# SketchyScene/SketchySceneColorization

Hardware: AMD Instinct MI355X
Metric: train images/sec (192x192, gen+disc fwd+bwd) (higher is better)
Workload: dtype fp32 (bf16x6 split on the bf16 MFMA, fp32 accumulate; filter gradients and few-channel layers on the exact-fp32 MFMA); 1 GPU; Foreground_Instance_Colorization Pix2Pix GAN train step (D-step + G-step, TF-Adam), 192x192, batch 32 per GPU; global_batch=32, parallelism=dp1, ranks_observed_by_allreduce=1, launcher=in-process, block_type=Pix2Pix, launch=hipGraph replay

## Files before the change

### sketchyscenecolorization_amd/csrc/igemm_bf16.hip

```cpp
#include <hip/hip_runtime.h>
#include <stdint.h>
#include <stdio.h>
#include <stdlib.h>
#include "sketchycolor_hip.h"
#include "igemm_util.h"
#include "igemm_epilogue.h"
#include "host_util.h"

#define BK 32
#ifndef SSC_BF_DIAG_BUILD
#define SSC_BF_DIAG_BUILD 0
#endif
typedef short bf16x8 __attribute__((ext_vector_type(8)));
typedef __bf16 bf16x2_t __attribute__((ext_vector_type(2)));
typedef unsigned u32x2_t __attribute__((ext_vector_type(2)));

__device__ unsigned g_sk_cfg_bf[4] = {2000000000u, 0u, 0u, 0u};

int ssc_sk_configure_bf(const unsigned* cfg4) {
    return (int)hipMemcpyToSymbol(HIP_SYMBOL(g_sk_cfg_bf), cfg4, 4 * sizeof(unsigned), 0, hipMemcpyHostToDevice);
}

template <int N>
__device__ __forceinline__ void glds16_run(const char* sbase, const unsigned* voff, unsigned lds_addr) {
    unsigned keep;
    if (N == 1) {
        asm volatile("s_mov_b32 %0, m0\n\ts_mov_b32 m0, %3\n\ts_nop 0\n\tglobal_load_lds_dwordx4 %1, %2\n\ts_mov_b32 m0, %0"
                     : "=&s"(keep) : "v"(voff[0]), "s"(sbase), "s"(lds_addr) : "memory");
    } else if (N == 2) {
        asm volatile("s_mov_b32 %0, m0\n\ts_mov_b32 m0, %4\n\ts_nop 0\n\tglobal_load_lds_dwordx4 %1, %3\n\t"
                     "s_add_u32 m0, m0, 0x400\n\ts_nop 0\n\tglobal_load_lds_dwordx4 %2, %3\n\ts_mov_b32 m0, %0"
                     : "=&s"(keep) : "v"(voff[0]), "v"(voff[1]), "s"(sbase), "s"(lds_addr) : "memory", "scc");
    } else {
        static_assert(N >= 1 && N <= 3, "1..3 instructions per run");
        asm volatile("s_mov_b32 %0, m0\n\ts_mov_b32 m0, %5\n\ts_nop 0\n\tglobal_load_lds_dwordx4 %1, %4\n\t"
                     "s_add_u32 m0, m0, 0x400\n\ts_nop 0\n\tglobal_load_lds_dwordx4 %2, %4\n\t"
                     "s_add_u32 m0, m0, 0x400\n\ts_nop 0\n\tglobal_load_lds_dwordx4 %3, %4\n\ts_mov_b32 m0, %0"
                     : "=&s"(keep) : "v"(voff[0]), "v"(voff[1]), "v"(voff[2]), "s"(sbase), "s"(lds_addr) : "memory", "scc");
    }
}

__device__ __forceinline__ unsigned cvt_pk_bf16(float a, float b) {
    const f32x2_t v = {a, b};
    return __builtin_bit_cast(unsigned, __builtin_convertvector(v, bf16x2_t));
}
__device__ __forceinline__ void split3_pair(float x0, float x1, unsigned& h, unsigned& m, unsigned& l) {
    if (SSC_BF_DIAG_BUILD & 16) { h = m = l = __float_as_uint(x0) ^ __float_as_uint(x1); return; }
    h = cvt_pk_bf16(x0, x1);
    const float r0 = x0 - __uint_as_float(h << 16), r1 = x1 - __uint_as_float(h & 0xffff0000u);
    m = cvt_pk_bf16(r0, r1);
    const float s0 = r0 - __uint_as_float(m << 16), s1 = r1 - __uint_as_float(m & 0xffff0000u);
    l = cvt_pk_bf16(s0, s1);
}

struct SplitGeom { int K, N, KC, NBP; };
static inline SplitGeom split_geom(int c0, int c1, int orient) {
    SplitGeom g;
    g.K = orient ? c1 : c0;
    g.N = orient ? c0 : c1;
    g.KC = 2 * ((g.K + 31) / 32);
    g.NBP = (g.N + 31) / 32 + 3;
    return g;
}

static int64_t ssc_filter_split_bytes(int taps, int c0, int c1, int orient) {
    const SplitGeom g = split_geom(c0, c1, orient);
    return (int64_t)taps * g.KC * 3 * g.NBP * 1024;
}

__device__ __forceinline__ unsigned rne_bf16_bits(float x) {
    const unsigned u = __float_as_uint(x);
    return (u + 0x7fffu + ((u >> 16) & 1u)) & 0xffff0000u;
}

__device__ __forceinline__ void filter_split_body(const ssc_split_job& jb, long lt) {
    const int K = jb.orient ? jb.c1 : jb.c0, N = jb.orient ? jb.c0 : jb.c1;
    const int KC = 2 * ((K + 31) / 32), NBP = (N + 31) / 32 + 3;
    const long nfrag = (long)jb.taps * KC * NBP;
    if (lt >= nfrag * 64) return;
    const int lane = (int)(lt & 63);
    const long f = lt >> 6;
    const int nb = (int)(f % NBP);
    const long r = f / NBP;
    const int kc = (int)(r % KC), tap = (int)(r / KC);
    const int n = nb * 32 + (lane & 31), k0 = kc * 16 + (lane >> 5) * 8;
    unsigned hb[8], mb[8], lb[8];
#pragma unroll
    for (int e = 0; e < 8; ++e) {
        const int k = k0 + e;
        float x = 0.f;
        if (k < K && n < N)
            x = jb.orient ? jb.w[((long)tap * jb.c0 + n) * jb.c1 + k] : jb.w[((long)tap * jb.c0 + k) * jb.c1 + n];
        const unsigned h = rne_bf16_bits(x);
        const float r1 = x - __uint_as_float(h);
        const unsigned m = rne_bf16_bits(r1);
        const float r2 = r1 - __uint_as_float(m);
        hb[e] = h; mb[e] = m; lb[e] = rne_bf16_bits(r2);
    }
    uint4 vh, vm, vl;
    vh.x = (hb[0] >> 16) | hb[1]; vh.y = (hb[2] >> 16) | hb[3]; vh.z = (hb[4] >> 16) | hb[5]; vh.w = (hb[6] >> 16) | hb[7];
    vm.x = (mb[0] >> 16) | mb[1]; vm.y = (mb[2] >> 16) | mb[3]; vm.z = (mb[4] >> 16) | mb[5]; vm.w = (mb[6] >> 16) | mb[7];
    vl.x = (lb[0] >> 16) | lb[1]; vl.y = (lb[2] >> 16) | lb[3]; vl.z = (lb[4] >> 16) | lb[5]; vl.w = (lb[6] >> 16) | lb[7];
    char* base = reinterpret_cast<char*>(jb.dst) + ((((long)tap * KC + kc) * 3) * NBP + nb) * 1024 + lane * 16;
    *reinterpret_cast<uint4*>(base) = vh;
    *reinterpret_cast<uint4*>(base + (long)NBP * 1024) = vm;
    *reinterpret_cast<uint4*>(base + (long)2 * NBP * 1024) = vl;
}

__global__ __launch_bounds__(256) void filter_split_kernel(const ssc_split_job* __restrict__ jobs, int njobs) {
    const long t = (long)blockIdx.x * 256 + threadIdx.x;
    const long tb = (long)blockIdx.x * 256;
    int lo = 0, hi = njobs - 1;
    while (lo < hi) {
        const int mid = (lo + hi + 1) >> 1;
        if (jobs[mid].first_thread <= tb) lo = mid;
        else hi = mid - 1;
    }
    const ssc_split_job jb = jobs[lo];
    filter_split_body(jb, t - jb.first_thread);
}
__global__ __launch_bounds__(256) void filter_split_one_kernel(const ssc_split_job jb) {
    filter_split_body(jb, (long)blockIdx.x * 256 + threadIdx.x);
}

static int64_t ssc_filter_split_threads(int taps, int c0, int c1, int orient) {
    const SplitGeom g = split_geom(c0, c1, orient);
    return (((int64_t)taps * g.KC * g.NBP * 64 + 255) / 256) * 256;
}

extern "C" int ssc_filter_split_geom(int taps, int c0, int c1, int orient, int* kc, int* nbp, int64_t* bytes, int64_t* threads) {
    if (taps <= 0 || c0 <= 0 || c1 <= 0) return -1;
    const SplitGeom g = split_geom(c0, c1, orient);
    if (kc) *kc = g.KC;
    if (nbp) *nbp = g.NBP;
    if (bytes) *bytes = ssc_filter_split_bytes(taps, c0, c1, orient);
    if (threads) *threads = ssc_filter_split_threads(taps, c0, c1, orient);
    return 0;
}

extern "C" int ssc_filter_split_batch(const ssc_split_job* jobs_dev, int njobs, int64_t total_threads, void* stream) {
    if (njobs <= 0 || total_threads <= 0) return 0;
    if (total_threads / 256 > 0x7fffffffL) return -1;
    hipLaunchKernelGGL(filter_split_kernel, dim3((unsigned)(total_threads / 256)), dim3(256), 0, (hipStream_t)stream, jobs_dev, njobs);
    return (int)hipGetLastError();
}

#define BF_A_RS 208
#define BF_WAIT_ALL() do { asm volatile("s_waitcnt vmcnt(0)" ::: "memory"); __builtin_amdgcn_s_waitcnt(0x0070); } while (0)
template <int BM, int BN, bool SS = false> struct BfLds {
    static constexpr int A_BYTES = BM * BF_A_RS;
    static constexpr int B_BYTES = 6 * (BN / 32) * 1024;
    static constexpr int EPI_BYTES = (BM * (BN + 4) + 2 * 256 * 4) * 4;
    static constexpr int ONE = A_BYTES + B_BYTES;
    static constexpr int OPER_BYTES = SS ? (ONE > EPI_BYTES ? ONE : EPI_BYTES) : 2 * ONE;
    static constexpr int TOTAL = OPER_BYTES + BM * 8;
};

struct BfTabs { const float* a0; const float* b0; const float* a1; const float* b1; };
template <int WM, int WN, int SM, int SN, bool PLAIN, bool ONE, bool KM = false, bool SS = false>
__global__ __launch_bounds__(256) void conv_bf_kernel(const ssc_conv_desc d, const Magics mg, float* __restrict__ slab_base,
                                                       long slab_stride, int splitk, int ts_full, int ts_s,
                                                       unsigned* __restrict__ flags, const BfTabs tab, const int korder) {
    constexpr int BM = WM * SM * 32;
    constexpr int BN = WN * SN * 32;
    constexpr int NBT = BN / 32;
    constexpr int A_BYTES = BfLds<BM, BN, SS>::A_BYTES, B_BYTES = BfLds<BM, BN, SS>::B_BYTES;
    constexpr int LDS_FLOATS = BfLds<BM, BN, SS>::OPER_BYTES / 4;
    constexpr int B_BASE = (SS ? 1 : 2) * A_BYTES;
    constexpr int A_ROWS = BM / 32;
    constexpr int B_IPW = 6 * NBT / 4;
    static_assert(WM * WN == 4 && (6 * NBT) % 4 == 0, "4 waves share the fragments of a K-tile evenly");

    extern __shared__ __attribute__((aligned(16))) float smem[];
    char* const sm_b = reinterpret_cast<char*>(smem);
    long* rowpix = reinterpret_cast<long*>(smem + LDS_FLOATS);

    const int tid = threadIdx.x;
    const int lane = tid & 63;
    const int wave = tid >> 6;
    const int wm = wave / WN, wn = wave % WN;
    const int l31 = lane & 31, lhi = lane >> 5;

    const float* const xs0 = d.x.s0;
    const float* const xs1 = d.x.s1;
    const int xC0 = d.x.C0, xC1 = d.x.C1, xH = d.x.H, xW = d.x.W;
    const int TWv = d.TW, kstep = d.kstep, KWv = d.KW;
    const float slope0 = act_slope(d.x.act), slope1 = act_slope(d.x.act1 >= 0 ? d.x.act1 : d.x.act);

    static_assert(!KM || ONE, "partial chunks: one source only");
    const int nch0 = KM ? (xC0 + BK - 1) / BK : xC0 / BK, nch1 = xC1 / BK;
    const int tpt = nch0 + nch1;
    const long M = (long)d.NB * d.PH * d.PW;
    const int PHW = d.PH * d.PW;
    int phase, ks, sk, n0, slot = 0;
    long m0;
    float* part = nullptr;
    if (ts_s > 0) {
        const int bid = blockIdx.x;
        int tile;
        if (bid < ts_full) {
            tile = bid; ks = 0; sk = 1;
        } else {
            const int r = bid - ts_full;
            const int q = r / (ts_s & 0xffff);
            tile = ts_full + q; ks = r - q * (ts_s & 0xffff); sk = ts_s & 0xffff;
            part = slab_base + (long)r * (BM * BN);
            slot = r;
        }
        const int mt = (int)((M + BM - 1) / BM), nt = (d.Nstore + BN - 1) / BN;
        if (ts_s & 0x10000) {
            if (bid < ts_full) tile = (bid & 7) * (ts_full >> 3) + (bid >> 3);
            const int r2 = tile / nt;
            n0 = (tile - r2 * nt) * BN;
            if (ts_s & 0x20000) {
                phase = r2 & 3;
                m0 = (long)(r2 >> 2) * BM;
            } else {
                phase = r2 / mt;
                m0 = (long)(r2 - phase * mt) * BM;
            }
            ts_s &= 0xffff;
            sk = bid < ts_full ? 1 : ts_s;
        } else {
            const int rest = tile / mt;
            m0 = (long)(tile - rest * mt) * BM;
            phase = rest / nt;
            n0 = (rest - phase * nt) * BN;
        }
    } else {
        phase = blockIdx.z / splitk;
        ks = blockIdx.z % splitk;
// ... 288 lines not shown
                        if (SSC_BF_DIAG_BUILD & 64) { asm volatile("" : "=v"(av[kc][i][p])); continue; }
                        av[kc][i][p] = *reinterpret_cast<const bf16x8*>(Ab + i * 32 * BF_A_RS + p * 64 + kc * 32);
                    }
            };
            auto fetch_b = [&](int kc) {
#pragma unroll
                for (int j = 0; j < SN; ++j)
#pragma unroll
                    for (int p = 0; p < 3; ++p) {
                        if (SSC_BF_DIAG_BUILD & 64) { asm volatile("" : "=v"(bv[kc][j][p])); continue; }
                        bv[kc][j][p] = *reinterpret_cast<const bf16x8*>(Bb + ((kc * 3 + p) * NBT + j) * 1024);
                    }
            };
            auto group = [&](int kc, int t) {
                if (SSC_BF_DIAG_BUILD & 1) return;
                constexpr int pa[6] = {2, 0, 1, 1, 0, 0}, pb[6] = {0, 2, 1, 0, 1, 0};
#pragma unroll
                for (int i = 0; i < SM; ++i)
#pragma unroll
                    for (int j = 0; j < SN; ++j) {
                        if (t == 5)
                            acc[i][j] = __builtin_amdgcn_mfma_f32_32x32x16_bf16(av[kc][i][0], bv[kc][j][0], acc[i][j], 0, 0, 0);
                        else
                            accc[i][j] = __builtin_amdgcn_mfma_f32_32x32x16_bf16(av[kc][i][pa[t]], bv[kc][j][pb[t]], accc[i][j], 0, 0, 0);
                    }
            };
#define BF_SB __builtin_amdgcn_sched_barrier(0)
            fetch_a(0);
            fetch_b(0);
            if (SS) {
                fetch_a(1);
                fetch_b(1);
                asm volatile("s_waitcnt lgkmcnt(0)" ::: "memory");
                __builtin_amdgcn_s_barrier();
            }
            BF_SB;
            float z0, w0, z1, w1;
            unsigned ha, ma, la, hb, mb, lb;
            group(0, 0); dma_b(td, nxt, 0); BF_SB;
            group(0, 1); if (RUN1 > 0) dma_b(td, nxt, 1); BF_SB;
            if (kt + 2 <= last) kt_advance(tl);
            group(0, 2); issue_loads(tl, SB); BF_SB;
            group(0, 3); if (!SS) fetch_a(1); BF_SB;
            group(0, 4); if (!SS) fetch_b(1); BF_SB;
            if (A_ROWS == 2) {
                group(0, 5); BF_STAGE_A(SA, 0, z0, w0, ha, ma, la); BF_SB;
                group(1, 0); BF_STAGE_B(nxt, 0, z0, w0, ha, ma, la); BF_SB;
                group(1, 1); BF_STAGE_A(SA, 1, z1, w1, hb, mb, lb); BF_SB;
                group(1, 2); BF_STAGE_B(nxt, 1, z1, w1, hb, mb, lb); BF_SB;
                group(1, 3); BF_SB;
                group(1, 4); BF_SB;
                group(1, 5); BF_SB;
            } else {
                group(0, 5); BF_STAGE_A(SA, 0, z0, w0, ha, ma, la); BF_SB;
                group(1, 0); BF_STAGE_B(nxt, 0, z0, w0, ha, ma, la); BF_STAGE_A(SA, 1, z1, w1, hb, mb, lb); BF_SB;
                group(1, 1); BF_STAGE_B(nxt, 1, z1, w1, hb, mb, lb); BF_STAGE_A(SA, 2, z0, w0, ha, ma, la); BF_SB;
                group(1, 2); BF_STAGE_B(nxt, 2, z0, w0, ha, ma, la); BF_STAGE_A(SA, 3, z1, w1, hb, mb, lb); BF_SB;
                group(1, 3); BF_STAGE_B(nxt, 3, z1, w1, hb, mb, lb); BF_SB;
                group(1, 4); BF_SB;
                group(1, 5); BF_SB;
            }
#undef BF_SB
            BF_WAIT_ALL();
            td = tl;
            __builtin_amdgcn_s_barrier();
        };
        for (int kt = kt_begin; kt < kt_end; kt += 2) {
            kstep(S0, S1, 0, kt);
            if (kt + 1 < kt_end) kstep(S1, S0, 1, kt + 1);
        }
    }

#pragma unroll
    for (int i = 0; i < SM; ++i)
#pragma unroll
        for (int j = 0; j < SN; ++j)
#pragma unroll
            for (int r = 0; r < 16; ++r) acc[i][j][r] += accc[i][j][r];
    ut_epilogue<BM, BN, WM, WN, SM, SN, LDS_FLOATS>(acc, d, smem, rowpix, part, ks, sk, slot, flags, ts_s, splitk, slab_base,
                                                   slab_stride, m0, n0, phase, M, g_sk_cfg_bf);
}

#define BFH_A_RS 112
template <int BM, int BN> struct BfhLds {
    static constexpr int A_BYTES = BM * BFH_A_RS;
    static constexpr int B_BYTES = 3 * (BN / 32) * 1024;
    static constexpr int OPER_BYTES = 2 * (A_BYTES + B_BYTES);
    static constexpr int EPI_BYTES = (BM * (BN + 4) + 2 * 256 * 4) * 4;
    static constexpr int LDS_BYTES = OPER_BYTES > EPI_BYTES ? OPER_BYTES : EPI_BYTES;
    static constexpr int TOTAL = LDS_BYTES + BM * 8;
};

template <int WM, int WN, bool PLAIN, bool ONE, bool KM = false>
__global__ __launch_bounds__(256, 2) void conv_bfh_kernel(const ssc_conv_desc d, const Magics mg, float* __restrict__ slab_base,
                                                           long slab_stride, int splitk, int ts_full, int ts_s,
                                                           unsigned* __restrict__ flags, const BfTabs tab, const int korder) {
    static_assert(WM * WN == 4, "four waves");
    constexpr int SM = 2, SN = 2, BM = WM * SM * 32, BN = WN * SN * 32, NBT = BN / 32, KS = 16;
    constexpr int A_BYTES = BfhLds<BM, BN>::A_BYTES, B_BYTES = BfhLds<BM, BN>::B_BYTES;
    constexpr int LDS_FLOATS = BfhLds<BM, BN>::LDS_BYTES / 4;
    constexpr int B_BASE = 2 * A_BYTES;
    constexpr int A_ROWS = BM / 64;
    constexpr int B_IPW = 3 * NBT / 4;

    extern __shared__ __attribute__((aligned(16))) float smem[];
    char* const sm_b = reinterpret_cast<char*>(smem);
    long* rowpix = reinterpret_cast<long*>(smem + LDS_FLOATS);

    const int tid = threadIdx.x;
    const int lane = tid & 63;
    const int wave = tid >> 6;
    const int wm = wave / WN, wn = wave % WN;
    const int l31 = lane & 31, lhi = lane >> 5;

    const float* const xs0 = d.x.s0;
    const float* const xs1 = d.x.s1;
    const int xC0 = d.x.C0, xC1 = d.x.C1, xH = d.x.H, xW = d.x.W;
    const int TWv = d.TW, kstep = d.kstep, KWv = d.KW;
    const float slope0 = act_slope(d.x.act), slope1 = act_slope(d.x.act1 >= 0 ? d.x.act1 : d.x.act);

    static_assert(!KM || ONE, "partial chunks: one source only");
    const int nch0 = KM ? (xC0 + KS - 1) / KS : xC0 / KS, nch1 = xC1 / KS;
    const int tpt = nch0 + nch1;
    const long M = (long)d.NB * d.PH * d.PW;
    const int PHW = d.PH * d.PW;
    int phase, ks, sk, n0, slot = 0;
    long m0;
    float* part = nullptr;
    if (ts_s > 0) {
        const int bid = blockIdx.x;
        int tile;
        if (bid < ts_full) {
            tile = bid; ks = 0; sk = 1;
        } else {
            const int r = bid - ts_full;
            const int q = r / (ts_s & 0xffff);
            tile = ts_full + q; ks = r - q * (ts_s & 0xffff); sk = ts_s & 0xffff;
            part = slab_base + (long)r * (BM * BN);
            slot = r;
        }
        const int mt = (int)((M + BM - 1) / BM), nt = (d.Nstore + BN - 1) / BN;
        if (ts_s & 0x10000) {
            if (bid < ts_full) tile = (bid & 7) * (ts_full >> 3) + (bid >> 3);
            const int r2 = tile / nt;
            n0 = (tile - r2 * nt) * BN;
            if (ts_s & 0x20000) {
                phase = r2 & 3;
                m0 = (long)(r2 >> 2) * BM;
            } else {
                phase = r2 / mt;
                m0 = (long)(r2 - phase * mt) * BM;
            }
            ts_s &= 0xffff;
            sk = bid < ts_full ? 1 : ts_s;
        } else {
            const int rest = tile / mt;
            m0 = (long)(tile - rest * mt) * BM;
            phase = rest / nt;
            n0 = (rest - phase * nt) * BN;
        }
    } else {
        phase = blockIdx.z / splitk;
        ks = blockIdx.z % splitk;
        sk = splitk;
        m0 = (long)blockIdx.x * BM;
        n0 = blockIdx.y * BN;
    }
    const FwdPhase ph = fwd_phase(d, phase);

    const int a_col4 = tid & 3;
    const int aq = tid >> 2;
    const int arow = (aq & ~7) | ((aq & 3) << 1) | ((aq >> 2) & 1);
    const bool a_lastv = !KM || (nch0 - 1) * KS + a_col4 * 4 < xC0;
    uint4 a_lastm = make_uint4(~0u, ~0u, ~0u, ~0u);
    if (KM) {
        const int c_ = (nch0 - 1) * KS + a_col4 * 4;
        a_lastm = make_uint4(c_ < d.k_real ? ~0u : 0u, c_ + 1 < d.k_real ? ~0u : 0u, c_ + 2 < d.k_real ? ~0u : 0u,
                             c_ + 3 < d.k_real ? ~0u : 0u);
    }
    int a_iyb[A_ROWS], a_ixb[A_ROWS], a_off0[A_ROWS], a_off1[A_ROWS];
    bool a_mv[A_ROWS];
#pragma unroll
    for (int i = 0; i < A_ROWS; ++i) {
        const int row = arow + 64 * i;
        const long m = m0 + row;
        a_mv[i] = m < M;
// ... 76 lines not shown
            if (korder == 1) {
                t.ty = sidx / TWv;
                t.tx = sidx - t.ty * TWv;
            } else {
                const int hw = TWv >> 1, pc = ntaps >> 2;
                const int cls = sidx / pc, j = sidx - cls * pc;
                const int jy = j / hw, jx = j - jy * hw;
                t.ty = 2 * jy + (cls >> 1);
                t.tx = 2 * jx + (cls & 1);
            }
            kt_place(t);
            return t;
        }
        const int tap = div32(kt, mg.mC, mg.oneC);
        t.chunk = kt - tap * tpt;
        t.ty = div32(tap, mg.mTW, mg.oneTW);
        t.tx = tap - t.ty * TWv;
        kt_place(t);
        return t;
    };
    const long W0 = (long)(ph.ky0 * KWv + ph.kx0) * KC * KB;
    const long SX2 = 2 * SX, DY2 = 2 * SY - (long)TWv * SX;
    auto kt_advance = [&](KTile& t) {
        if (korder == 1) {
            t.tx += 1;
            t.tapidx += 1;
            t.tappix += 1;
            t.woff += SX;
            if (t.tx == TWv) {
                t.tx = 0;
                t.ty += 1;
                t.tappix += xW - TWv;
                t.woff += DY;
                if (t.ty == THv) {
                    t.ty = 0;
                    t.chunk += 1;
                    t.tapidx = 0;
                    t.tappix = 0;
                    t.woff = W0 + (long)t.chunk * KB;
                }
            }
            return;
        }
        if (korder == 2) {
            t.tx += 2;
            t.tapidx += 2;
            t.tappix += 2;
            t.woff += SX2;
            if (t.tx >= TWv) {
                t.tx -= TWv;
                t.ty += 2;
                t.tapidx += TWv;
                t.tappix += 2 * xW - TWv;
                t.woff += DY2;
                if (t.ty >= THv) {
                    t.ty &= 1;
                    if (t.tx == 0) t.tx = 1;
                    else {
                        t.tx = 0;
                        if (t.ty == 0) t.ty = 1;
                        else { t.ty = 0; t.chunk += 1; }
                    }
                    kt_place(t);
                }
            }
            return;
        }
        t.chunk += 1;
        t.woff += KB;
        if (t.chunk == tpt) {
            t.chunk = 0;
            t.tx += 1;
            t.tapidx += 1;
            t.tappix += 1;
            t.woff += DX;
            if (t.tx == TWv) {
                t.tx = 0;
                t.tappix += xW - TWv;
                t.woff += DY;
            }
        }
    };

    struct ASet { float4 r[A_ROWS]; float v[A_ROWS]; float4 aa, ab; float slope; uint4 km; };
    auto issue_loads = [&](const KTile& t, ASet& S) {
        const bool first = ONE ? true : t.chunk < nch0;
        const int cs = first ? xC0 : xC1;
        const int cc = (first ? t.chunk : t.chunk - nch0) * KS;
        const char* sbase = reinterpret_cast<const char*>((first ? xs0 : xs1) + cc);
        const int tapshift = t.tappix * cs * 4;
        const int tapidx = t.tapidx;
        const bool cv = !KM || t.chunk != nch0 - 1 || a_lastv;
        if (KM) S.km = t.chunk == nch0 - 1 ? a_lastm : make_uint4(~0u, ~0u, ~0u, ~0u);
        if (!PLAIN) {
            const char* pa = reinterpret_cast<const char*>((first ? tab.a0 : tab.a1) + cc);
            const char* pb = reinterpret_cast<const char*>((first ? tab.b0 : tab.b1) + cc);
            const int tc = (KM && !cv) ? 0 : a_col4 * 16;
            S.aa = *reinterpret_cast<const float4*>(pa + tc);
            S.ab = *reinterpret_cast<const float4*>(pb + tc);
            S.slope = first ? slope0 : slope1;
        }
#pragma unroll
        for (int i = 0; i < A_ROWS; ++i) {
            const unsigned vb = cv ? (a_vm[i] >> tapidx) & 1u : 0u;
            const int osel = first ? a_off0[i] : a_off1[i];
            const unsigned off = vb ? (unsigned)(osel + tapshift) : (unsigned)(a_col4 * 16);
            S.v[i] = (float)vb;
            S.r[i] = *reinterpret_cast<const float4*>(sbase + off);
        }
    };
    auto dma_b = [&](const KTile& t, int buf) {
        const unsigned dst = __builtin_amdgcn_readfirstlane((unsigned)(B_BASE + buf * B_BYTES + wave * B_IPW * 1024));
        glds16_run<3>(wsp + t.woff, bd_off, dst);
        if (B_IPW == 6) glds16_run<3>(wsp + t.woff, bd_off + 3, dst + 3 * 1024);
    };
#define BFH_STAGE_A(S, i, Z, W, H0, M0, L0)                                                       \
    do {                                                                                          \
        float4 v_ = (S).r[i];                                                                     \
        if (PLAIN) {                                                                              \
            v_.x *= (S).v[i]; v_.y *= (S).v[i]; v_.z *= (S).v[i]; v_.w *= (S).v[i];               \
        } else {                                                                                  \
            float t_;                                                                             \
            t_ = fmaf((S).aa.x, v_.x, (S).ab.x); v_.x = fmaxf(t_, t_ * (S).slope) * (S).v[i];     \
            t_ = fmaf((S).aa.y, v_.y, (S).ab.y); v_.y = fmaxf(t_, t_ * (S).slope) * (S).v[i];     \
            t_ = fmaf((S).aa.z, v_.z, (S).ab.z); v_.z = fmaxf(t_, t_ * (S).slope) * (S).v[i];     \
            t_ = fmaf((S).aa.w, v_.w, (S).ab.w); v_.w = fmaxf(t_, t_ * (S).slope) * (S).v[i];     \
        }                                                                                         \
        if (KM) {                                                                                 \
            v_.x = __uint_as_float(__float_as_uint(v_.x) & (S).km.x);                             \
            v_.y = __uint_as_float(__float_as_uint(v_.y) & (S).km.y);                             \
            v_.z = __uint_as_float(__float_as_uint(v_.z) & (S).km.z);                             \
            v_.w = __uint_as_float(__float_as_uint(v_.w) & (S).km.w);                             \
        }                                                                                         \
        split3_pair(v_.x, v_.y, H0, M0, L0);                                                      \
        Z = v_.z; W = v_.w;                                                                       \
    } while (0)
#define BFH_STAGE_B(buf, i, Z, W, H0, M0, L0)                                                     \
    do {                                                                                          \
        unsigned h1_, m1_, l1_;                                                                   \
        split3_pair(Z, W, h1_, m1_, l1_);                                                         \
        char* p_ = sm_b + (buf) * A_BYTES + (arow + 64 * (i)) * BFH_A_RS + a_col4 * 8;            \
        *reinterpret_cast<uint2*>(p_) = make_uint2(H0, h1_);                                      \
        *reinterpret_cast<uint2*>(p_ + 32) = make_uint2(M0, m1_);                                 \
        *reinterpret_cast<uint2*>(p_ + 64) = make_uint2(L0, l1_);                                 \
    } while (0)

    if (kt_begin < kt_end) {
        const int last = kt_end - 1;
        ASet S0, S1;
        KTile tl = kt_decode(kt_begin);
        dma_b(tl, 0);
        issue_loads(tl, S0);
#pragma unroll
        for (int i = 0; i < A_ROWS; ++i) {
            float z, w;
            unsigned h0, m0_, l0;
            BFH_STAGE_A(S0, i, z, w, h0, m0_, l0);
            BFH_STAGE_B(0, i, z, w, h0, m0_, l0);
        }
        KTile td = tl;
        if (kt_begin + 1 <= last) kt_advance(tl);
        td = tl;
        issue_loads(tl, S0);
        BF_WAIT_ALL();
        __builtin_amdgcn_s_barrier();
        auto kstep = [&](ASet& SA, ASet& SB, const int cur, const int kt) {
            const int nxt = cur ^ 1;
            const char* Ab = sm_b + cur * A_BYTES + (wm * SM * 32 + l31) * BFH_A_RS + lhi * 16;
            const char* Bb = sm_b + B_BASE + cur * B_BYTES + (wn * SN) * 1024 + lane * 16;
            bf16x8 av[SM][3], bv[SN][3];
#pragma unroll
            for (int i = 0; i < SM; ++i)
#pragma unroll
                for (int p = 0; p < 3; ++p) av[i][p] = *reinterpret_cast<const bf16x8*>(Ab + i * 32 * BFH_A_RS + p * 32);
#pragma unroll
            for (int j = 0; j < SN; ++j)
#pragma unroll
                for (int p = 0; p < 3; ++p) bv[j][p] = *reinterpret_cast<const bf16x8*>(Bb + (p * NBT + j) * 1024);
            auto group = [&](int t) {
                constexpr int pa[6] = {2, 0, 1, 1, 0, 0}, pb[6] = {0, 2, 1, 0, 1, 0};
#pragma unroll
                for (int i = 0; i < SM; ++i)
#pragma unroll
                    for (int j = 0; j < SN; ++j) {
                        if (t == 5) acc[i][j] = __builtin_amdgcn_mfma_f32_32x32x16_bf16(av[i][0], bv[j][0], acc[i][j], 0, 0, 0);
                        else accc[i][j] = __builtin_amdgcn_mfma_f32_32x32x16_bf16(av[i][pa[t]], bv[j][pb[t]], accc[i][j], 0, 0, 0);
                    }
            };
#define BFH_SB __builtin_amdgcn_sched_barrier(0)
            BFH_SB;
            float z0, w0, z1, w1;
            unsigned ha, ma, la, hb, mb, lb;
            group(0); dma_b(td, nxt); BFH_SB;
            if (kt + 2 <= last) kt_advance(tl);
            group(1); issue_loads(tl, SB); BFH_SB;
            group(2); BFH_STAGE_A(SA, 0, z0, w0, ha, ma, la); BFH_SB;
            group(3); BFH_STAGE_B(nxt, 0, z0, w0, ha, ma, la); BFH_SB;
            if (A_ROWS == 2) {
                group(4); BFH_STAGE_A(SA, A_ROWS - 1, z1, w1, hb, mb, lb); BFH_SB;
                group(5); BFH_STAGE_B(nxt, A_ROWS - 1, z1, w1, hb, mb, lb); BFH_SB;
            } else {
                group(4); BFH_SB;
                group(5); BFH_SB;
            }
#undef BFH_SB
            BF_WAIT_ALL();
            td = tl;
            __builtin_amdgcn_s_barrier();
        };
        for (int kt = kt_begin; kt < kt_end; kt += 2) {
            kstep(S0, S1, 0, kt);
            if (kt + 1 < kt_end) kstep(S1, S0, 1, kt + 1);
        }
    }
#undef BFH_STAGE_A
#undef BFH_STAGE_B

#pragma unroll
    for (int i = 0; i < SM; ++i)
#pragma unroll
        for (int j = 0; j < SN; ++j)
#pragma unroll
            for (int r = 0; r < 16; ++r) acc[i][j][r] += accc[i][j][r];
    ut_epilogue<BM, BN, WM, WN, SM, SN, LDS_FLOATS>(acc, d, smem, rowpix, part, ks, sk, slot, flags, ts_s, splitk, slab_base,
                                                   slab_stride, m0, n0, phase, M, g_sk_cfg_bf);
}

#ifdef SSC_ISA_ONLY
template __global__ void conv_bf_kernel<2, 2, 1, 2, false, true>(const ssc_conv_desc, const Magics, float*, long, int, int, int, unsigned*, const BfTabs, const int);
template __global__ void conv_bf_kernel<2, 2, 1, 2, false, false>(const ssc_conv_desc, const Magics, float*, long, int, int, int, unsigned*, const BfTabs, const int);
#else
void ssc_launch_slab_reduce(const float* ws, long out_count, int splitk, const ssc_conv_desc& d, hipStream_t st);

#define BF_IDENT_C 4096
static const float* bf_identity_rows() {
    static float* rows[16] = {nullptr};
    int dev = 0;
    if (hipGetDevice(&dev) != hipSuccess || dev < 0 || dev >= 16) return nullptr;
    if (rows[dev] == nullptr) {
        float* p = nullptr;
        if (hipMalloc(&p, 2 * BF_IDENT_C * sizeof(float)) != hipSuccess) return nullptr;
        float* h = (float*)malloc(2 * BF_IDENT_C * sizeof(float));
        for (int i = 0; i < BF_IDENT_C; ++i) { h[i] = 1.f; h[BF_IDENT_C + i] = 0.f; }
        const hipError_t e = hipMemcpy(p, h, 2 * BF_IDENT_C * sizeof(float), hipMemcpyHostToDevice);
        free(h);
        if (e != hipSuccess) return nullptr;
        rows[dev] = p;
    }
    return rows[dev];
}
extern "C" int ssc_bf16_prepare(void) { return bf_identity_rows() != nullptr ? 0 : -1; }

static bool bf_tabs(const ssc_conv_desc& d, BfTabs& t) {
    const float* id = bf_identity_rows();
    if (id == nullptr || d.x.C0 > BF_IDENT_C || d.x.C1 > BF_IDENT_C) return false;
    t.a0 = d.x.ab0 ? d.x.ab0 : id;
    t.b0 = d.x.ab0 ? d.x.ab0 + d.x.C0 : id + BF_IDENT_C;
    t.a1 = d.x.ab1 ? d.x.ab1 : id;
    t.b1 = d.x.ab1 ? d.x.ab1 + d.x.C1 : id + BF_IDENT_C;
    return true;
}

template <int WM, int WN, int SM, int SN, bool PLAIN, bool ONE, bool KM = false, bool SS = false>
static int launch_bf_t(const ssc_conv_desc& d, int splitk, float* ws, hipStream_t st, long ts_full, int ts_s, int64_t ws_bytes,
                       int xcd) {
    constexpr int BM = WM * SM * 32, BN = WN * SN * 32;
    constexpr size_t lds = BfLds<BM, BN, SS>::TOTAL;
    const long M = (long)d.NB * d.PH * d.PW;
    const int tpt = (d.x.C0 + BK - 1) / BK + d.x.C1 / BK;
    const Magics mg = make_magics((unsigned)tpt, (unsigned)d.TW, (unsigned long)d.PW, (unsigned long)d.PH * d.PW, (unsigned long)M);
    const long mt = (M + BM - 1) / BM;
    const int nt = (d.Nstore + BN - 1) / BN;
    const long out_count = (long)d.NB * d.OH * d.OW * d.ldc;
    static unsigned long long attr_done = 0;
    {
        const int arc = ssc_set_max_lds(reinterpret_cast<const void*>(&conv_bf_kernel<WM, WN, SM, SN, PLAIN, ONE, KM, SS>), (int)lds, &attr_done);
        if (arc != 0) return arc;
    }
    BfTabs tab = {nullptr, nullptr, nullptr, nullptr};
    if (!PLAIN && !bf_tabs(d, tab)) return -5;
    const int xflag = 0x10000 | ((xcd >= 2 && d.nphase == 4) ? 0x20000 : 0);
    static int diag = -1;
    if (diag < 0) {
        const char* e = ssc_dev_getenv("SSC_BF_DIAG");
        diag = e != nullptr ? atoi(e) : 0;
    }
    if (diag & 2) xcd = 0;
    static int kord = -2;
    if (kord == -2) {
        const char* e = ssc_dev_getenv("SSC_BF_KORDER");
        kord = e != nullptr ? atoi(e) : -1;
    }
    const bool par_ok = d.in_stride == 2 && (d.TH & 1) == 0 && (d.TW & 1) == 0;
    int korder = par_ok ? 2 : 1;
    if (kord >= 0) korder = (kord == 2 && !par_ok) ? 1 : kord;
    if (d.TH * d.TW == 1) korder = 0;
    if (!(diag & 1) && splitk == 1 && ws != nullptr && d.sk_flags != nullptr && ts_s > 1) {
        const long tiles = mt * nt * d.nphase;
        const long full = ts_full, tail = tiles - full, s = ts_s;
        if (full >= 0 && tail > 0 && (int64_t)tail * s * BM * BN * 4 <= ws_bytes && tail * s < SSC_SK_FLAG_WORDS - 1 &&
            full + tail * s < 0x7fffffffL) {
            hipLaunchKernelGGL((conv_bf_kernel<WM, WN, SM, SN, PLAIN, ONE, KM, SS>), dim3((unsigned)(full + tail * s)), dim3(256), lds, st, d, mg,
                               ws, out_count, 1, (int)full, (int)s | ((xcd && (full & 7) == 0) ? xflag : 0), d.sk_flags, tab, korder);
            return (int)hipGetLastError();
        }
    }
    if (splitk == 1 && xcd) {
        const long tiles = mt * nt * d.nphase;
        const long full = tiles & ~7L;
        if (tiles < 0x7fffffffL && full > 0) {
            hipLaunchKernelGGL((conv_bf_kernel<WM, WN, SM, SN, PLAIN, ONE, KM, SS>), dim3((unsigned)tiles), dim3(256), lds, st, d, mg, ws,
                               out_count, 1, (int)full, 1 | xflag, (unsigned*)nullptr, tab, korder);
            return (int)hipGetLastError();
        }
    }
    dim3 grid((unsigned)mt, (unsigned)nt, (unsigned)(d.nphase * splitk));
    hipLaunchKernelGGL((conv_bf_kernel<WM, WN, SM, SN, PLAIN, ONE, KM, SS>), grid, dim3(256), lds, st, d, mg, ws, out_count, splitk, 0, 0,
                       (unsigned*)nullptr, tab, korder);
    if (splitk > 1) ssc_launch_slab_reduce(ws, out_count, splitk, d, st);
    return (int)hipGetLastError();
}

template <int WM, int WN, bool PLAIN, bool ONE, bool KM = false>
static int launch_bfh_t(const ssc_conv_desc& d, int splitk, float* ws, hipStream_t st, long ts_full, int ts_s, int64_t ws_bytes,
                        int xcd) {
    constexpr int BM = WM * 64, BN = WN * 64;
    constexpr size_t lds = BfhLds<BM, BN>::TOTAL;
    const long M = (long)d.NB * d.PH * d.PW;
    const int tpt = (d.x.C0 + 15) / 16 + d.x.C1 / 16;
    const Magics mg = make_magics((unsigned)tpt, (unsigned)d.TW, (unsigned long)d.PW, (unsigned long)d.PH * d.PW, (unsigned long)M);
    const long mt = (M + BM - 1) / BM;
    const int nt = (d.Nstore + BN - 1) / BN;
    const long out_count = (long)d.NB * d.OH * d.OW * d.ldc;
    static unsigned long long attr_done = 0;
    {
        const int arc = ssc_set_max_lds(reinterpret_cast<const void*>(&conv_bfh_kernel<WM, WN, PLAIN, ONE, KM>), (int)lds, &attr_done);
        if (arc != 0) return arc;
    }
    BfTabs tab = {nullptr, nullptr, nullptr, nullptr};
    if (!PLAIN && !bf_tabs(d, tab)) return -5;
    const int xflag = 0x10000 | ((xcd >= 2 && d.nphase == 4) ? 0x20000 : 0);
    const bool par_ok = d.in_stride == 2 && (d.TH & 1) == 0 && (d.TW & 1) == 0;
    int korder = par_ok ? 2 : 1;
    if (d.TH * d.TW == 1) korder = 0;
    if (splitk == 1 && ws != nullptr && d.sk_flags != nullptr && ts_s > 1) {
        const long tiles = mt * nt * d.nphase;
        const long full = ts_full, tail = tiles - full, s = ts_s;
        if (full >= 0 && tail > 0 && (int64_t)tail * s * BM * BN * 4 <= ws_bytes && tail * s < SSC_SK_FLAG_WORDS - 1 &&
            full + tail * s < 0x7fffffffL) {
            hipLaunchKernelGGL((conv_bfh_kernel<WM, WN, PLAIN, ONE, KM>), dim3((unsigned)(full + tail * s)), dim3(256), lds, st, d, mg, ws, out_count,
                               1, (int)full, (int)s | ((xcd && (full & 7) == 0) ? xflag : 0), d.sk_flags, tab, korder);
            return (int)hipGetLastError();
        }
    }
    if (splitk == 1 && xcd) {
        const long tiles = mt * nt * d.nphase;
        const long full = tiles & ~7L;
        if (tiles < 0x7fffffffL && full > 0) {
            hipLaunchKernelGGL((conv_bfh_kernel<WM, WN, PLAIN, ONE, KM>), dim3((unsigned)tiles), dim3(256), lds, st, d, mg, ws, out_count, 1,
                               (int)full, 1 | xflag, (unsigned*)nullptr, tab, korder);
            return (int)hipGetLastError();
        }
    }
    dim3 grid((unsigned)mt, (unsigned)nt, (unsigned)(d.nphase * splitk));
    hipLaunchKernelGGL((conv_bfh_kernel<WM, WN, PLAIN, ONE, KM>), grid, dim3(256), lds, st, d, mg, ws, out_count, splitk, 0, 0, (unsigned*)nullptr,
                       tab, korder);
    if (splitk > 1) ssc_launch_slab_reduce(ws, out_count, splitk, d, st);
    return (int)hipGetLastError();
}

template <int WM, int WN, int SM, int SN, bool SS>
static int launch_bf_form(bool plain, bool one, bool km, const ssc_conv_desc& d, int splitk, float* ws, hipStream_t st, long ts_full,
                          int ts_s, int64_t ws_bytes, int xcd) {
    if (km) return plain ? launch_bf_t<WM, WN, SM, SN, true, true, true, SS>(d, splitk, ws, st, ts_full, ts_s, ws_bytes, xcd)
                         : launch_bf_t<WM, WN, SM, SN, false, true, true, SS>(d, splitk, ws, st, ts_full, ts_s, ws_bytes, xcd);
    return one ? (plain ? launch_bf_t<WM, WN, SM, SN, true, true, false, SS>(d, splitk, ws, st, ts_full, ts_s, ws_bytes, xcd)
                        : launch_bf_t<WM, WN, SM, SN, false, true, false, SS>(d, splitk, ws, st, ts_full, ts_s, ws_bytes, xcd))
               : (plain ? launch_bf_t<WM, WN, SM, SN, true, false, false, SS>(d, splitk, ws, st, ts_full, ts_s, ws_bytes, xcd)
                        : launch_bf_t<WM, WN, SM, SN, false, false, false, SS>(d, splitk, ws, st, ts_full, ts_s, ws_bytes, xcd));
}

bool ssc_bf_hk_enabled() {
    static int hk_env = -2;
    if (hk_env == -2) {
        const char* e = ssc_dev_getenv("SSC_BF_HK");
        hk_env = e != nullptr ? (e[0] == '1' ? 1 : 0) : -1;
    }
    return hk_env != 0;
}

int ssc_launch_conv_bf(int cfg, bool plain, const ssc_conv_desc& d, int splitk, float* ws, hipStream_t st, long ts_full, int ts_s,
                       int64_t ws_bytes, int xcd) {
    const bool one = d.x.C1 == 0;
    const bool km = one && (d.x.C0 % BK) != 0;
    static int ss_env = -2;
    if (ss_env == -2) {
        const char* e = ssc_dev_getenv("SSC_BF_SS");
        ss_env = e != nullptr ? (e[0] == '1' ? 1 : 0) : -1;
    }
    const bool ss = ss_env >= 0 ? ss_env == 1 : (d.lds_hint & 1) != 0;
#define BF_CASE(WM, WN, SM, SN)                                                                                              \
    return ss ? launch_bf_form<WM, WN, SM, SN, true>(plain, one, km, d, splitk, ws, st, ts_full, ts_s, ws_bytes, xcd)         \
              : launch_bf_form<WM, WN, SM, SN, false>(plain, one, km, d, splitk, ws, st, ts_full, ts_s, ws_bytes, xcd)
#define BFH_CASE(WMV, WNV)                                                                                        \
    if (km) return plain ? launch_bfh_t<WMV, WNV, true, true, true>(d, splitk, ws, st, ts_full, ts_s, ws_bytes, xcd)     \
                         : launch_bfh_t<WMV, WNV, false, true, true>(d, splitk, ws, st, ts_full, ts_s, ws_bytes, xcd);   \
    return one ? (plain ? launch_bfh_t<WMV, WNV, true, true>(d, splitk, ws, st, ts_full, ts_s, ws_bytes, xcd)        \
                        : launch_bfh_t<WMV, WNV, false, true>(d, splitk, ws, st, ts_full, ts_s, ws_bytes, xcd))      \
               : (plain ? launch_bfh_t<WMV, WNV, true, false>(d, splitk, ws, st, ts_full, ts_s, ws_bytes, xcd)       \
                        : launch_bfh_t<WMV, WNV, false, false>(d, splitk, ws, st, ts_full, ts_s, ws_bytes, xcd))
    if (cfg == 0 && ssc_bf_hk_enabled()) {
        BFH_CASE(2, 2);
    }
#undef BFH_CASE
    switch (cfg) {
        case 0: return launch_bf_form<2, 2, 2, 2, false>(plain, one, km, d, splitk, ws, st, ts_full, ts_s, ws_bytes, xcd);
        case 1: BF_CASE(2, 2, 1, 2);
        case 2: BF_CASE(2, 2, 2, 1);
        case 4: BF_CASE(2, 2, 1, 1);
        default: return -4;
    }
#undef BF_CASE
}

extern "C" int ssc_filter_split(const float* w, int taps, int c0, int c1, int orient, void* dst, void* stream) {
    ssc_split_job jb;
    jb.w = w; jb.dst = dst; jb.taps = taps; jb.c0 = c0; jb.c1 = c1; jb.orient = orient; jb.first_thread = 0;
    const int64_t threads = ssc_filter_split_threads(taps, c0, c1, orient);
    if (threads / 256 > 0x7fffffffL) return -1;
    hipLaunchKernelGGL(filter_split_one_kernel, dim3((unsigned)(threads / 256)), dim3(256), 0, (hipStream_t)stream, jb);
    return (int)hipGetLastError();
}
#endif
```

Measured before the change: 2377 images/sec.

## Triple-buffer B operand and use counted vmcnt waits in bfh conv kernel

```diff
diff --git a/sketchyscenecolorization_amd/csrc/igemm_bf16.hip b/sketchyscenecolorization_amd/csrc/igemm_bf16.hip
--- a/sketchyscenecolorization_amd/csrc/igemm_bf16.hip
+++ b/sketchyscenecolorization_amd/csrc/igemm_bf16.hip
@@ -14,6 +14,7 @@
 typedef short bf16x8 __attribute__((ext_vector_type(8)));
 typedef __bf16 bf16x2_t __attribute__((ext_vector_type(2)));
 typedef unsigned u32x2_t __attribute__((ext_vector_type(2)));
+typedef float f32x4_t __attribute__((ext_vector_type(4)));
 
 __device__ unsigned g_sk_cfg_bf[4] = {2000000000u, 0u, 0u, 0u};
 
@@ -147,6 +148,11 @@
 
 #define BF_A_RS 208
 #define BF_WAIT_ALL() do { asm volatile("s_waitcnt vmcnt(0)" ::: "memory"); __builtin_amdgcn_s_waitcnt(0x0070); } while (0)
+__device__ __forceinline__ f32x4_t gload16_raw(const char* sbase, unsigned voff) {
+    f32x4_t r;
+    asm volatile("global_load_dwordx4 %0, %1, %2" : "=v"(r) : "v"(voff), "s"(sbase));
+    return r;
+}
 template <int BM, int BN, bool SS = false> struct BfLds {
     static constexpr int A_BYTES = BM * BF_A_RS;
     static constexpr int B_BYTES = 6 * (BN / 32) * 1024;
@@ -601,26 +607,27 @@
 }
 
 #define BFH_A_RS 112
-template <int BM, int BN> struct BfhLds {
+template <int BM, int BN, bool H3 = false> struct BfhLds {
     static constexpr int A_BYTES = BM * BFH_A_RS;
     static constexpr int B_BYTES = 3 * (BN / 32) * 1024;
-    static constexpr int OPER_BYTES = 2 * (A_BYTES + B_BYTES);
+    static constexpr int OPER_BYTES = 2 * A_BYTES + (H3 ? 3 : 2) * B_BYTES;
     static constexpr int EPI_BYTES = (BM * (BN + 4) + 2 * 256 * 4) * 4;
     static constexpr int LDS_BYTES = OPER_BYTES > EPI_BYTES ? OPER_BYTES : EPI_BYTES;
     static constexpr int TOTAL = LDS_BYTES + BM * 8;
 };
 
-template <int WM, int WN, bool PLAIN, bool ONE, bool KM = false>
+template <int WM, int WN, bool PLAIN, bool ONE, bool KM = false, bool H3 = true>
 __global__ __launch_bounds__(256, 2) void conv_bfh_kernel(const ssc_conv_desc d, const Magics mg, float* __restrict__ slab_base,
                                                            long slab_stride, int splitk, int ts_full, int ts_s,
                                                            unsigned* __restrict__ flags, const BfTabs tab, const int korder) {
     static_assert(WM * WN == 4, "four waves");
     constexpr int SM = 2, SN = 2, BM = WM * SM * 32, BN = WN * SN * 32, NBT = BN / 32, KS = 16;
-    constexpr int A_BYTES = BfhLds<BM, BN>::A_BYTES, B_BYTES = BfhLds<BM, BN>::B_BYTES;
-    constexpr int LDS_FLOATS = BfhLds<BM, BN>::LDS_BYTES / 4;
+    constexpr int A_BYTES = BfhLds<BM, BN, H3>::A_BYTES, B_BYTES = BfhLds<BM, BN, H3>::B_BYTES;
+    constexpr int LDS_FLOATS = BfhLds<BM, BN, H3>::LDS_BYTES / 4;
     constexpr int B_BASE = 2 * A_BYTES;
     constexpr int A_ROWS = BM / 64;
     constexpr int B_IPW = 3 * NBT / 4;
+    static_assert(!H3 || A_ROWS == 2, "H3: BFH_VM_WAIT names two staged rows");
 
     extern __shared__ __attribute__((aligned(16))) float smem[];
     char* const sm_b = reinterpret_cast<char*>(smem);
@@ -863,7 +870,7 @@
         }
     };
 
-    struct ASet { float4 r[A_ROWS]; float v[A_ROWS]; float4 aa, ab; float slope; uint4 km; };
+    struct ASet { f32x4_t r[A_ROWS]; float v[A_ROWS]; f32x4_t aa, ab; float slope; uint4 km; };
     auto issue_loads = [&](const KTile& t, ASet& S) {
         const bool first = ONE ? true : t.chunk < nch0;
         const int cs = first ? xC0 : xC1;
@@ -877,8 +884,13 @@
             const char* pa = reinterpret_cast<const char*>((first ? tab.a0 : tab.a1) + cc);
             const char* pb = reinterpret_cast<const char*>((first ? tab.b0 : tab.b1) + cc);
             const int tc = (KM && !cv) ? 0 : a_col4 * 16;
-            S.aa = *reinterpret_cast<const float4*>(pa + tc);
-            S.ab = *reinterpret_cast<const float4*>(pb + tc);
+            if (H3) {
+                S.aa = gload16_raw(pa, (unsigned)tc);
+                S.ab = gload16_raw(pb, (unsigned)tc);
+            } else {
+                S.aa = *reinterpret_cast<const f32x4_t*>(pa + tc);
+                S.ab = *reinterpret_cast<const f32x4_t*>(pb + tc);
+            }
             S.slope = first ? slope0 : slope1;
         }
 #pragma unroll
@@ -887,9 +899,16 @@
             const int osel = first ? a_off0[i] : a_off1[i];
             const unsigned off = vb ? (unsigned)(osel + tapshift) : (unsigned)(a_col4 * 16);
             S.v[i] = (float)vb;
-            S.r[i] = *reinterpret_cast<const float4*>(sbase + off);
+            if (H3) S.r[i] = gload16_raw(sbase, off);
+            else S.r[i] = *reinterpret_cast<const f32x4_t*>(sbase + off);
         }
     };
+    constexpr int VM_DMA = B_IPW, VM_LOADS = A_ROWS + (PLAIN ? 0 : 2);
+#define BFH_VM_WAIT(N, S)                                                                                                   \
+    do {                                                                                                                    \
+        if (PLAIN) asm volatile("s_waitcnt vmcnt(%2)" : "+v"((S).r[0]), "+v"((S).r[1]) : "n"(N) : "memory");                \
+        else asm volatile("s_waitcnt vmcnt(%4)" : "+v"((S).r[0]), "+v"((S).r[1]), "+v"((S).aa), "+v"((S).ab) : "n"(N) : "memory"); \
+    } while (0)
     auto dma_b = [&](const KTile& t, int buf) {
         const unsigned dst = __builtin_amdgcn_readfirstlane((unsigned)(B_BASE + buf * B_BYTES + wave * B_IPW * 1024));
         glds16_run<3>(wsp + t.woff, bd_off, dst);
@@ -897,7 +916,7 @@
     };
 #define BFH_STAGE_A(S, i, Z, W, H0, M0, L0)                                                       \
     do {                                                                                          \
-        float4 v_ = (S).r[i];                                                                     \
+        f32x4_t v_ = (S).r[i];                                                                    \
         if (PLAIN) {                                                                              \
             v_.x *= (S).v[i]; v_.y *= (S).v[i]; v_.z *= (S).v[i]; v_.w *= (S).v[i];               \
         } else {                                                                                  \
@@ -932,6 +951,7 @@
         KTile tl = kt_decode(kt_begin);
         dma_b(tl, 0);
         issue_loads(tl, S0);
+        if constexpr (H3) BFH_VM_WAIT(0, S0);
 #pragma unroll
         for (int i = 0; i < A_ROWS; ++i) {
             float z, w;
@@ -942,13 +962,15 @@
         KTile td = tl;
         if (kt_begin + 1 <= last) kt_advance(tl);
         td = tl;
+        if constexpr (H3) dma_b(tl, 1);
         issue_loads(tl, S0);
-        BF_WAIT_ALL();
+        if constexpr (H3) asm volatile("s_waitcnt lgkmcnt(0)" ::: "memory");
+        else BF_WAIT_ALL();
         __builtin_amdgcn_s_barrier();
-        auto kstep = [&](ASet& SA, ASet& SB, const int cur, const int kt) {
+        auto kstep = [&](ASet& SA, ASet& SB, const int cur, const int kt, const int bc) {
             const int nxt = cur ^ 1;
             const char* Ab = sm_b + cur * A_BYTES + (wm * SM * 32 + l31) * BFH_A_RS + lhi * 16;
-            const char* Bb = sm_b + B_BASE + cur * B_BYTES + (wn * SN) * 1024 + lane * 16;
+            const char* Bb = sm_b + B_BASE + (H3 ? bc : cur) * B_BYTES + (wn * SN) * 1024 + lane * 16;
             bf16x8 av[SM][3], bv[SN][3];
 #pragma unroll
             for (int i = 0; i < SM; ++i)
@@ -972,9 +994,16 @@
             BFH_SB;
             float z0, w0, z1, w1;
             unsigned ha, ma, la, hb, mb, lb;
-            group(0); dma_b(td, nxt); BFH_SB;
-            if (kt + 2 <= last) kt_advance(tl);
-            group(1); issue_loads(tl, SB); BFH_SB;
+            if constexpr (H3) {
+                if (kt + 2 <= last) kt_advance(tl);
+                group(0); dma_b(tl, bc == 0 ? 2 : bc - 1); BFH_SB;
+                group(1); issue_loads(tl, SB); BFH_SB;
+                BFH_VM_WAIT(VM_DMA + VM_LOADS, SA);
+            } else {
+                group(0); dma_b(td, nxt); BFH_SB;
+                if (kt + 2 <= last) kt_advance(tl);
+                group(1); issue_loads(tl, SB); BFH_SB;
+            }
             group(2); BFH_STAGE_A(SA, 0, z0, w0, ha, ma, la); BFH_SB;
             group(3); BFH_STAGE_B(nxt, 0, z0, w0, ha, ma, la); BFH_SB;
             if (A_ROWS == 2) {
@@ -985,17 +1014,27 @@
                 group(5); BFH_SB;
             }
 #undef BFH_SB
-            BF_WAIT_ALL();
+            if constexpr (H3) asm volatile("s_waitcnt lgkmcnt(0)" ::: "memory");
+            else BF_WAIT_ALL();
             td = tl;
             __builtin_amdgcn_s_barrier();
         };
+        int bc = 0;
         for (int kt = kt_begin; kt < kt_end; kt += 2) {
-            kstep(S0, S1, 0, kt);
-            if (kt + 1 < kt_end) kstep(S1, S0, 1, kt + 1);
+            kstep(S0, S1, 0, kt, bc);
+            bc = bc == 2 ? 0 : bc + 1;
+            if (kt + 1 < kt_end) kstep(S1, S0, 1, kt + 1, bc);
+            bc = bc == 2 ? 0 : bc + 1;
+        }
+        if constexpr (H3) {
+            BFH_VM_WAIT(0, S0);
+            BFH_VM_WAIT(0, S1);
+            __builtin_amdgcn_s_barrier();
         }
     }
 #undef BFH_STAGE_A
 #undef BFH_STAGE_B
+#undef BFH_VM_WAIT
 
 #pragma unroll
     for (int i = 0; i < SM; ++i)
@@ -1102,11 +1141,11 @@
     return (int)hipGetLastError();
 }
 
-template <int WM, int WN, bool PLAIN, bool ONE, bool KM = false>
+template <int WM, int WN, bool PLAIN, bool ONE, bool KM, bool H3>
 static int launch_bfh_t(const ssc_conv_desc& d, int splitk, float* ws, hipStream_t st, long ts_full, int ts_s, int64_t ws_bytes,
                         int xcd) {
     constexpr int BM = WM * 64, BN = WN * 64;
-    constexpr size_t lds = BfhLds<BM, BN>::TOTAL;
+    constexpr size_t lds = BfhLds<BM, BN, H3>::TOTAL;
     const long M = (long)d.NB * d.PH * d.PW;
     const int tpt = (d.x.C0 + 15) / 16 + d.x.C1 / 16;
     const Magics mg = make_magics((unsigned)tpt, (unsigned)d.TW, (unsigned long)d.PW, (unsigned long)d.PH * d.PW, (unsigned long)M);
@@ -1115,7 +1154,7 @@
     const long out_count = (long)d.NB * d.OH * d.OW * d.ldc;
     static unsigned long long attr_done = 0;
     {
-        const int arc = ssc_set_max_lds(reinterpret_cast<const void*>(&conv_bfh_kernel<WM, WN, PLAIN, ONE, KM>), (int)lds, &attr_done);
+        const int arc = ssc_set_max_lds(reinterpret_cast<const void*>(&conv_bfh_kernel<WM, WN, PLAIN, ONE, KM, H3>), (int)lds, &attr_done);
         if (arc != 0) return arc;
     }
     BfTabs tab = {nullptr, nullptr, nullptr, nullptr};
@@ -1129,7 +1168,7 @@
         const long full = ts_full, tail = tiles - full, s = ts_s;
         if (full >= 0 && tail > 0 && (int64_t)tail * s * BM * BN * 4 <= ws_bytes && tail * s < SSC_SK_FLAG_WORDS - 1 &&
             full + tail * s < 0x7fffffffL) {
-            hipLaunchKernelGGL((conv_bfh_kernel<WM, WN, PLAIN, ONE, KM>), dim3((unsigned)(full + tail * s)), dim3(256), lds, st, d, mg, ws, out_count,
+            hipLaunchKernelGGL((conv_bfh_kernel<WM, WN, PLAIN, ONE, KM, H3>), dim3((unsigned)(full + tail * s)), dim3(256), lds, st, d, mg, ws, out_count,
                                1, (int)full, (int)s | ((xcd && (full & 7) == 0) ? xflag : 0), d.sk_flags, tab, korder);
             return (int)hipGetLastError();
         }
@@ -1138,13 +1177,13 @@
         const long tiles = mt * nt * d.nphase;
         const long full = tiles & ~7L;
         if (tiles < 0x7fffffffL && full > 0) {
-            hipLaunchKernelGGL((conv_bfh_kernel<WM, WN, PLAIN, ONE, KM>), dim3((unsigned)tiles), dim3(256), lds, st, d, mg, ws, out_count, 1,
+            hipLaunchKernelGGL((conv_bfh_kernel<WM, WN, PLAIN, ONE, KM, H3>), dim3((unsigned)tiles), dim3(256), lds, st, d, mg, ws, out_count, 1,
                                (int)full, 1 | xflag, (unsigned*)nullptr, tab, korder);
             return (int)hipGetLastError();
         }
     }
     dim3 grid((unsigned)mt, (unsigned)nt, (unsigned)(d.nphase * splitk));
-    hipLaunchKernelGGL((conv_bfh_kernel<WM, WN, PLAIN, ONE, KM>), grid, dim3(256), lds, st, d, mg, ws, out_count, splitk, 0, 0, (unsigned*)nullptr,
+    hipLaunchKernelGGL((conv_bfh_kernel<WM, WN, PLAIN, ONE, KM, H3>), grid, dim3(256), lds, st, d, mg, ws, out_count, splitk, 0, 0, (unsigned*)nullptr,
                        tab, korder);
     if (splitk > 1) ssc_launch_slab_reduce(ws, out_count, splitk, d, st);
     return (int)hipGetLastError();
@@ -1170,6 +1209,15 @@
     return hk_env != 0;
 }
 
+static bool ssc_bf_hk3_enabled() {
+    static int env = -2;
+    if (env == -2) {
+        const char* e = ssc_dev_getenv("SSC_BF_HK3");
+        env = e != nullptr ? (e[0] == '1' ? 1 : 0) : -1;
+    }
+    return env != 0;
+}
+
 int ssc_launch_conv_bf(int cfg, bool plain, const ssc_conv_desc& d, int splitk, float* ws, hipStream_t st, long ts_full, int ts_s,
                        int64_t ws_bytes, int xcd) {
     const bool one = d.x.C1 == 0;
@@ -1183,15 +1231,18 @@
 #define BF_CASE(WM, WN, SM, SN)                                                                                              \
     return ss ? launch_bf_form<WM, WN, SM, SN, true>(plain, one, km, d, splitk, ws, st, ts_full, ts_s, ws_bytes, xcd)         \
               : launch_bf_form<WM, WN, SM, SN, false>(plain, one, km, d, splitk, ws, st, ts_full, ts_s, ws_bytes, xcd)
-#define BFH_CASE(WMV, WNV)                                                                                        \
-    if (km) return plain ? launch_bfh_t<WMV, WNV, true, true, true>(d, splitk, ws, st, ts_full, ts_s, ws_bytes, xcd)     \
-                         : launch_bfh_t<WMV, WNV, false, true, true>(d, splitk, ws, st, ts_full, ts_s, ws_bytes, xcd);   \
-    return one ? (plain ? launch_bfh_t<WMV, WNV, true, true>(d, splitk, ws, st, ts_full, ts_s, ws_bytes, xcd)        \
-                        : launch_bfh_t<WMV, WNV, false, true>(d, splitk, ws, st, ts_full, ts_s, ws_bytes, xcd))      \
-               : (plain ? launch_bfh_t<WMV, WNV, true, false>(d, splitk, ws, st, ts_full, ts_s, ws_bytes, xcd)       \
-                        : launch_bfh_t<WMV, WNV, false, false>(d, splitk, ws, st, ts_full, ts_s, ws_bytes, xcd))
+#define BFH_CASE(WMV, WNV, H3)                                                                                         \
+    if (km) return plain ? launch_bfh_t<WMV, WNV, true, true, true, H3>(d, splitk, ws, st, ts_full, ts_s, ws_bytes, xcd)      \
+                         : launch_bfh_t<WMV, WNV, false, true, true, H3>(d, splitk, ws, st, ts_full, ts_s, ws_bytes, xcd);    \
+    return one ? (plain ? launch_bfh_t<WMV, WNV, true, true, false, H3>(d, splitk, ws, st, ts_full, ts_s, ws_bytes, xcd)      \
+                        : launch_bfh_t<WMV, WNV, false, true, false, H3>(d, splitk, ws, st, ts_full, ts_s, ws_bytes, xcd))    \
+               : (plain ? launch_bfh_t<WMV, WNV, true, false, false, H3>(d, splitk, ws, st, ts_full, ts_s, ws_bytes, xcd)     \
+                        : launch_bfh_t<WMV, WNV, false, false, false, H3>(d, splitk, ws, st, ts_full, ts_s, ws_bytes, xcd))
     if (cfg == 0 && ssc_bf_hk_enabled()) {
-        BFH_CASE(2, 2);
+        if (ssc_bf_hk3_enabled()) {
+            BFH_CASE(2, 2, true);
+        }
+        BFH_CASE(2, 2, false);
     }
 #undef BFH_CASE
     switch (cfg) {
```

New measurement: 2364 images/sec (median of 2 runs). No clear change (-0.6%).
